# KarelPeeters/kZero

Measured on AMD Instinct MI355X. Metric: self-play NN evals/sec (node), Chess 20x256 ResNet b=256, 1/2/4/8 GPU, higher is better.
Workload: dtype f16; 1 GPU; chess-20x256 attention head, executor batch 256; engines_per_gpu=1, parallelism=dp1 (no collective)

## Files before the change

kzero_amd/csrc/kz_device_weights.hpp:

```cpp
#pragma once

struct DevConv {
    void *w = nullptr;
    float *b = nullptr;
    int cin_p = 0, cout_p = 0, cout = 0, k = 1;
    void *bw = nullptr;
    bool bw2 = false;
    void *bws = nullptr;
    void *sw = nullptr;
};

struct DeviceWeights {
    int device = 0, dtype = 0;
    std::vector<void *> allocs;

    std::vector<DevConv> tower;
    float *post_scale = nullptr, *post_shift = nullptr;

    bool split16 = false;
    float *h32_small = nullptr;
    void *res32_w = nullptr;
    void *res_w_stem = nullptr, *res_w_tower = nullptr;
    float *res_bias = nullptr;
    int32_t *att_idx = nullptr;
// ... 186 lines not shown
                upload_f32(m.att_embedding, &att_embedding))
                return 1;
        } else if (p.tower == Tower::att_valu) {
            std::vector<float> all;
            all.reserve(kz::att_tower_layer_elems(C, m.att_heads, m.att_dk, m.att_dv, m.att_dff) * m.att_layers.size());
            for (auto &l : m.att_layers) {
                all.insert(all.end(), l.qkv.begin(), l.qkv.end());
                all.insert(all.end(), l.out.begin(), l.out.end());
                all.insert(all.end(), l.ff0.begin(), l.ff0.end());
                all.insert(all.end(), l.ff1.begin(), l.ff1.end());
            }
            if (upload_f32(m.att_expand, &att_expand) || upload_f32(m.att_embedding, &att_embedding) || upload_f32(all, &att_layers)) return 1;
        } else if (p.tower == Tower::resident_split16 || p.tower == Tower::resident_f16g) {
            const bool conv_heads = p.heads && m.policy_kind != kz::POLICY_ATTENTION;
            const bool heads = p.heads && !conv_heads;
            const size_t tower_elems = kz::tower_split_weight_elems(C, m.depth, m.c_in, split16);
            std::vector<uint16_t> packed(tower_elems + (heads ? kz::tower_split_heads_weight_elems() : 0) +
                                         (conv_heads ? kz::tower_split_conv_heads_weight_elems(C, split16) : 0));
            const size_t step_elems = (size_t)(split16 ? 2 : 1) * C * 32, stem_elems = kz::tower_split_stem_elems(C, m.c_in, split16),
                         layer_elems = (size_t)9 * (C / 32) * step_elems;
            kz::tower_split_pack_weights(m.tower[0].w.data(), C, m.c_in, hw, true, split16, packed.data());
            for (int l = 0; l < 2 * m.depth; l++)
                kz::tower_split_pack_weights(m.tower[1 + l].w.data(), C, C, hw, false, split16,
                                             packed.data() + stem_elems + layer_elems * l);
            std::vector<float> bias((size_t)(1 + 2 * m.depth + (heads ? 5 : conv_heads ? 1 : 0)) * C);
            for (int l = 0; l < 1 + 2 * m.depth; l++)
                for (int o = 0; o < C; o++) bias[(size_t)l * C + o] = m.tower[l].b[o];
            if (conv_heads) {
                kz::tower_split_pack_conv_heads(m.p_conv0.w.data(), C, split16, packed.data() + tower_elems);
                for (int o = 0; o < C; o++) bias[(size_t)(1 + 2 * m.depth) * C + o] = m.p_conv0.b[o];
                if (!split16) {
                    std::vector<uint16_t> small(kz::tower_split_small_weight16_elems(C));
                    kz::tower_split_pack_small_weights16(m.sh_conv.w.data(), m.sh_conv.cout,
                                                         m.policy_extra_moves ? m.p_extra_conv.w.data() : nullptr,
                                                         m.p_conv1.w.data(), m.policy_conv_channels, C, small.data());
                    if (upload(small.data(), small.size() * 2, (void **)&h32_small)) return 1;
                } else {
                    std::vector<float> small(kz::tower32_small_weight_elems(C));
                    kz::tower32_pack_small_weights(m.sh_conv.w.data(), m.sh_conv.cout,
                                                   m.policy_extra_moves ? m.p_extra_conv.w.data() : nullptr, m.p_conv1.w.data(),
                                                   m.policy_conv_channels, C, small.data());
                    if (upload_f32(small, &h32_small)) return 1;
                }
            }
            if (heads) {
                kz::tower_split_pack_heads(m.p_bulk.w.data(), m.p_bulk.b.data(), m.p_under.w.data(), m.p_under.b.data(),
                                           packed.data() + tower_elems, bias.data() + (size_t)(1 + 2 * m.depth) * C);
                std::vector<int32_t> idx(m.flat_to_att.size());
                for (size_t i = 0; i < idx.size(); i++) idx[i] = (m.flat_to_att[i] / 88) * 96 + m.flat_to_att[i] % 88;
                if (upload(idx.data(), idx.size() * 4, (void **)&att_idx)) return 1;
            }
            if (upload(packed.data(), packed.size() * 2, &res32_w)) return 1;
            if (upload_f32(bias, &res_bias)) return 1;
        } else if (p.tower == Tower::resident_f32) {
            const bool heads32 = kz::tower32_heads_supported((int)m.policy_kind, m.policy_extra_moves,
                                                             m.policy_conv_channels, m.h, m.w, C, m.sh_conv.cout, m.sh_fc0.out);
            const size_t tower_elems = kz::tower32_weight_elems(m.c_in, C, m.depth);
            std::vector<float> packed(tower_elems + (heads32 ? kz::tower32_heads_weight_elems(C) : 0) +
                                      kz::tower32_weight_pad_elems(C), 0.0f);
            const size_t stem_elems = (size_t)9 * ((m.c_in + 15) / 16) * 16 * C, layer_elems = (size_t)9 * C * C;
            kz::tower32_pack_weights(m.tower[0].w.data(), C, m.c_in, true, packed.data());
            for (int l = 0; l < 2 * m.depth; l++)
                kz::tower32_pack_weights(m.tower[1 + l].w.data(), C, C, false, packed.data() + stem_elems + layer_elems * l);
            std::vector<float> bias((size_t)(1 + 2 * m.depth + (heads32 ? 1 : 0)) * C);
            for (int l = 0; l < 1 + 2 * m.depth; l++)
                for (int o = 0; o < C; o++) bias[(size_t)l * C + o] = m.tower[l].b[o];
            if (heads32) {
                kz::tower32_pack_head_weights(m.p_conv0.w.data(), C, packed.data() + tower_elems);
                for (int o = 0; o < C; o++) bias[(size_t)(1 + 2 * m.depth) * C + o] = m.p_conv0.b[o];
                std::vector<float> small(kz::tower32_small_weight_elems(C));
                kz::tower32_pack_small_weights(m.sh_conv.w.data(), m.sh_conv.cout,
                                               m.policy_extra_moves ? m.p_extra_conv.w.data() : nullptr, m.p_conv1.w.data(),
                                               m.policy_conv_channels, C, small.data());
                if (upload_f32(small, &h32_small)) return 1;
            }
            if (upload(packed.data(), packed.size() * 4, &res32_w)) return 1;
            if (upload_f32(bias, &res_bias)) return 1;
        } else if (p.tower == Tower::resident_f16) {
            const int cin_p = round_up(m.c_in, 32);
            const size_t stem_elems = (size_t)9 * 256 * cin_p, layer_elems = (size_t)9 * 256 * 256;
            const size_t head_elems = p.heads ? kz::tower_heads_weight_elems() : 0;
            std::vector<uint16_t> stem(stem_elems), rest(layer_elems * 2 * m.depth + head_elems + kz::tower_weight_pad_elems());
            kz::tower_pack_weights(m.tower[0].w.data(), C, m.c_in, cin_p, stem.data());
            for (int l = 0; l < 2 * m.depth; l++)
                kz::tower_pack_weights(m.tower[1 + l].w.data(), C, C, 256, rest.data() + layer_elems * l);
            std::vector<float> bias((size_t)(1 + 2 * m.depth + (p.heads ? 5 : 0)) * 256);
            for (int l = 0; l < 1 + 2 * m.depth; l++)
                for (int o = 0; o < 256; o++) bias[(size_t)l * 256 + o] = m.tower[l].b[o];
            if (p.heads) {
                kz::tower_pack_heads(m.p_bulk.w.data(), m.p_bulk.b.data(), m.p_under.w.data(), m.p_under.b.data(),
                                     rest.data() + layer_elems * 2 * m.depth, bias.data() + (size_t)(1 + 2 * m.depth) * 256);
                std::vector<int32_t> idx(m.flat_to_att.size());
                for (size_t i = 0; i < idx.size(); i++) idx[i] = (m.flat_to_att[i] / 88) * 96 + m.flat_to_att[i] % 88;
                if (upload(idx.data(), idx.size() * 4, (void **)&att_idx)) return 1;
            }
            if (upload(stem.data(), stem.size() * 2, &res_w_stem)) return 1;
            if (upload(rest.data(), rest.size() * 2, &res_w_tower)) return 1;
            if (upload_f32(bias, &res_bias)) return 1;
        } else {
            tower.resize(m.tower.size());
            const bool on = p.tower == Tower::board_conv_f16, use_board_split = p.tower == Tower::board_conv_split16;
#ifdef KZ_EXPERIMENTS
            conv2 = p.conv2;
            if (conv2) {
                std::vector<int> rowmap;
                std::vector<unsigned short> halo;
                kz::board_conv2_tables(m.h, m.w, rowmap, halo);
                bc_n_halo = (int)halo.size();
                if (upload(rowmap.data(), rowmap.size() * sizeof(int), (void **)&bc_rowmap)) return 1;
                if (upload(halo.data(), halo.size() * sizeof(unsigned short), (void **)&bc_halo)) return 1;
            }
#endif
            for (size_t i = 0; i < m.tower.size(); i++) {
                const bool stem64 = on && i == 0 && !conv2 && m.tower[0].cin <= 64 && m.tower[0].k == 3 &&
                                    kz::board_conv_supported(dtype, m.h, m.w, 64, m.tower[0].cout);
                const bool board = on && kz::board_conv_supported(dtype, m.h, m.w, m.tower[i].cin, m.tower[i].cout);
                if (use_board_split && i == 0 && m.tower[0].cin <= 32 && m.tower[0].k == 3) {
                    stem_split = true;
                    if (upload_board_conv_split(m.tower[0], tower[0], 32)) return 1;
                } else if (use_board_split && i >= 1) {
                    if (upload_board_conv_split(m.tower[i], tower[i])) return 1;
                } else if (stem64) {
                    stem_cin_p = 64;
                    if (upload_board_conv(m.tower[0], tower[0], 64)) return 1;
                } else if (board ? upload_board_conv(m.tower[i], tower[i]) : upload_conv(m.tower[i], tower[i])) {
                    return 1;
                }
            }
        }

        if (upload_f32(m.sh_conv.w, &sh_w0) || upload_f32(m.sh_conv.b, &sh_b0) || upload_f32(m.sh_fc0.w, &sh_w1) ||
            upload_f32(m.sh_fc0.b, &sh_b1) || upload_f32(m.sh_fc1.w, &sh_w2) || upload_f32(m.sh_fc1.b, &sh_b2))
            return 1;
        {
            std::vector<float> wt((size_t)m.sh_fc0.in * m.sh_fc0.out);
            for (int o = 0; o < m.sh_fc0.out; o++)
                for (int i = 0; i < m.sh_fc0.in; i++) wt[(size_t)i * m.sh_fc0.out + o] = m.sh_fc0.w[(size_t)o * m.sh_fc0.in + i];
            if (upload_f32(wt, &sh_w1t)) return 1;
        }

        if (p.tower == Tower::resident_f16 && p.heads) return 0;
        switch (m.policy_kind) {
            case kz::POLICY_ATAXX_CONV:
            case kz::POLICY_CONV:
                if (upload_conv(m.p_conv0, p_conv0)) return 1;
                if (upload_f32(m.p_conv1.w, &p_w1) || upload_f32(m.p_conv1.b, &p_b1)) return 1;
                if (m.policy_extra_moves) {
                    if (upload_f32(m.p_extra_conv.w, &pe_wc) || upload_f32(m.p_extra_conv.b, &pe_bc) ||
                        upload_f32(m.p_extra_fc.w, &pe_wl) || upload_f32(m.p_extra_fc.b, &pe_bl))
                        return 1;
                    if (m.sh_conv.cout == 4 && m.p_extra_conv.cout == 1 && m.p_extra_conv.cin == m.sh_conv.cin) {
                        std::vector<float> w0x(m.sh_conv.w);
                        w0x.insert(w0x.end(), m.p_extra_conv.w.begin(), m.p_extra_conv.w.end());
                        if (upload_f32(w0x, &sh_w0x)) return 1;
                    }
                }
                break;
            case kz::POLICY_ARIMAA: {
                if (upload_conv(m.p_conv0, p_conv0)) return 1;
                if (upload_f32(m.p_conv1.w, &p_w1) || upload_f32(m.p_conv1.b, &p_b1)) return 1;
                if (upload_f32(m.pa_conv.w, &pa_w0) || upload_f32(m.pa_conv.b, &pa_b0) || upload_f32(m.pa_fc0.w, &pa_w1) ||
                    upload_f32(m.pa_fc0.b, &pa_b1) || upload_f32(m.pa_fc1.w, &pa_w2) || upload_f32(m.pa_fc1.b, &pa_b2))
                    return 1;
                std::vector<float> wt((size_t)m.pa_fc0.in * m.pa_fc0.out);
                for (int o = 0; o < m.pa_fc0.out; o++)
                    for (int i = 0; i < m.pa_fc0.in; i++) wt[(size_t)i * m.pa_fc0.out + o] = m.pa_fc0.w[(size_t)o * m.pa_fc0.in + i];
                if (upload_f32(wt, &pa_w1t)) return 1;
                break;
            }
            case kz::POLICY_ATTENTION:
                if (p.att_heads) {
                    const int Q = m.policy_query_channels;
                    std::vector<uint16_t> packed(kz::att_heads_weight_elems(C, Q));
                    std::vector<float> bias((size_t)5 * Q + 16);
                    kz::att_heads_pack(m.p_bulk.w.data(), m.p_bulk.b.data(), m.p_under.w.data(), m.p_under.b.data(), m.sh_conv.w.data(),
                                       m.sh_conv.b.data(), C, Q, m.sh_conv.cout, packed.data(), bias.data());
                    if (upload(packed.data(), packed.size() * 2, &ah_w) || upload_f32(bias, &ah_bias)) return 1;
                } else if (upload_conv(m.p_bulk, p_bulk) || upload_conv(m.p_under, p_under)) {
                    return 1;
                }
                if (upload(m.flat_to_att.data(), m.flat_to_att.size() * 4, (void **)&flat_to_att)) return 1;
                break;
            case kz::POLICY_NONE: break;
            case kz::POLICY_DENSE: {
                int ch = C, ch_p = cp;
                if (m.dense_hidden_channels) {
                    if (upload_conv(m.p_conv0, p_conv0)) return 1;
                    ch = m.dense_hidden_channels;
                    ch_p = p_conv0.cout_p;
                }
                if (m.dense_hidden_size) {
                    if (upload_flat_linear(m.p_fc0, ch, hw, ch_p, p_fc0)) return 1;
                    if (upload_linear(m.p_fc1, p_fc1)) return 1;
                } else {
                    if (upload_flat_linear(m.p_fc1, ch, hw, ch_p, p_fc1)) return 1;
                }
                break;
            }
        }
        return 0;
    }
};

struct WeightsKey {
    const Model *model;
    int device, dtype;
    Tower tower;
    bool heads, att_heads, conv2 = false;
    WeightsKey(const Model *m, int device, int dtype, const PathPlan &p)
        : model(m), device(device), dtype(dtype), tower(p.tower), heads(p.heads && p.tower != Tower::resident_f32), att_heads(p.att_heads) {
#ifdef KZ_EXPERIMENTS
        conv2 = p.conv2;
#endif
    }
    auto fields() const { return std::tie(model, device, dtype, tower, heads, att_heads, conv2); }
    bool operator<(const WeightsKey &o) const { return fields() < o.fields(); }
};
std::mutex g_cache_mutex;
std::map<WeightsKey, std::weak_ptr<DeviceWeights>> g_cache;
```

kzero_amd/csrc/kz_kernels.hpp:

```cpp
#pragma once
#include <vector>
#include <hip/hip_runtime.h>

#include <cstdint>

namespace kz {

inline int round_up(int v, int m) { return (v + m - 1) / m * m; }

struct PackedBoards {
    const uint8_t *bits = nullptr;
    size_t stride = 0;
    const float *scalars = nullptr;
    int n_scalar = 0, n_bool = 0;
    int n_sym = 0;
    const uint8_t *sym = nullptr;
    const int32_t *square_src = nullptr;
};

void launch_encode_packed(int dtype, const PackedBoards &in, int batch, int hw, void *x, int ldx, hipStream_t stream);
void launch_encode_dense(int dtype, const float *nchw, int batch, int c, int hw, void *x, int ldx,
                         hipStream_t stream);

struct ConvArgs {
// ... 210 lines not shown
bool tower32_supported(int dtype, int h, int w, int channels, int depth);
bool tower32_dense3_supported(int policy_kind, int extra_moves, int pc, int h, int w, int channels, int hc, int hs, bool heads);
bool tower32_heads_supported(int policy_kind, int extra_moves, int pc, int h, int w, int channels, int hc, int hs);
bool conv_heads_fit(int nt, int policy_kind, int extra_moves, int pc, int h, int w, int channels, int hc, int hs,
                    size_t scratch_bytes = 0);
constexpr size_t F16_TAIL_SCRATCH_BYTES = 16 * 1024;
size_t tower32_small_weight_elems(int channels);
void tower32_pack_small_weights(const float *sh_w0, int hc, const float *pe_wc , const float *p_w1, int pc,
                                int channels, float *dst);
size_t tower32_heads_weight_elems(int channels);
void tower32_pack_head_weights(const float *oi, int channels, float *dst);
int tower32_boards_per_workgroup(int h, int w, int channels);
size_t tower32_weight_elems(int c_in, int channels, int depth);
size_t tower32_weight_pad_elems(int channels);
void tower32_pack_weights(const float *oihw, int cout, int cin, bool stem, float *dst);
void launch_tower32(const Tower32Args &a, hipStream_t stream);

bool tower_split_supported(int h, int w, int channels, int depth, int c_in, bool split);
int tower_split_boards_per_workgroup(int h, int w, int channels, bool split, int wide_batch = 0);
bool tower_split_wide_supported(int h, int w, int channels, int max_batch);
size_t tower_split_stem_elems(int channels, int c_in, bool split);
size_t tower_split_weight_elems(int channels, int depth, int c_in, bool split);
void tower_split_pack_weights(const float *oihw, int cout, int cin, int hw, bool stem, bool split, uint16_t *dst);
void launch_tower_split(const Tower32Args &a, hipStream_t stream);
bool tower_split_heads_supported(int policy_kind, int query_channels, int policy_len, int h, int w, int channels, int sh_channels,
                                 int sh_size);
size_t tower_split_heads_weight_elems();
void tower_split_pack_heads(const float *w_bulk, const float *b_bulk, const float *w_under, const float *b_under, uint16_t *dst,
                            float *bias5 );
bool tower_split_conv_heads_supported(int policy_kind, int extra_moves, int pc, int h, int w, int channels, int hc, int hs,
                                      bool split, int wide_batch = 0);
size_t tower_split_small_weight16_elems(int channels);
void tower_split_pack_small_weights16(const float *sh_w0, int hc, const float *pe_wc , const float *p_w1, int pc,
                                      int channels, uint16_t *dst);
size_t tower_split_conv_heads_weight_elems(int channels, bool split);
void tower_split_pack_conv_heads(const float *w , int channels, bool split, uint16_t *dst);
void launch_tower_pairs(const Tower32Args &a, bool split, hipStream_t stream);

struct Conv1x1SplitArgs {
    const void *x;
    int ldx;
    const void *weights;
    const float *bias;
    void *y;
    int ldy, M, cin_p, cout_p, relu, group, src_group, src_off;
    bool split;
    const float *pw1 = nullptr, *pb1 = nullptr;
    float *policy = nullptr;
    int policy_len = 0, hw = 0;
};
bool conv1x1_split_supported(int cin_p, int cout_p);
bool conv1x1_policy_epilogue_supported(int cin_p, int cout_p, int cout, int policy_channels);
size_t conv1x1_split_weight_elems(int cin_p, int cout_p, bool split);
void conv1x1_split_pack_weights(const float *w, int cout, int cin, int cout_p, int cin_p, bool split, uint16_t *dst);
void launch_conv1x1_split(const Conv1x1SplitArgs &a, hipStream_t stream);

struct TowerArgs {
    const void *x0;
    int cin_p;
    PackedBoards in;
    const void *w_stem;
    const void *w_tower;
    const float *bias;
    const float *post_scale, *post_shift;
    void *y;
    int batch, h, w, depth;
    int boards_per_wg;
    bool fused_heads;
    const float *sh_w0, *sh_b0, *sh_w1, *sh_b1, *sh_w2, *sh_b2;
    const int32_t *att_idx;
    float *scalars, *policy;
    int *nonfinite_flag;
    int epoch;
    DecodeArgs decode;
    bool prev;
};
bool tower_resident_supported(int dtype, int h, int w, int channels, int depth, int c_in);
bool tower_heads_supported(int policy_kind, int query_channels, int policy_len, int sh_channels, int sh_size);
size_t tower_packed_weight_elems(int cin_p, int depth);
size_t tower_heads_weight_elems();
size_t tower_weight_pad_elems();
void tower_pack_heads(const float *w_bulk, const float *b_bulk, const float *w_under, const float *b_under,
                      uint16_t *dst, float *bias5);
void tower_pack_weights(const float *oihw, int cout, int cin, int cin_p, uint16_t *dst);
void launch_tower_resident(const TowerArgs &a, hipStream_t stream);
size_t tower4_scratch_bytes(int batch);
void launch_tower_resident4(const TowerArgs &a, void *xres, hipStream_t stream);

}
```

kzero_amd/csrc/kz_tower.hip:

```cpp
#include <cstdlib>
#include <type_traits>
#include <vector>

#include "kz_kernels.hpp"
#include "kz_launch.hpp"

namespace kz {

typedef _Float16 h16;
typedef h16 h16x8 __attribute__((ext_vector_type(8)));
typedef h16 h16x4 __attribute__((ext_vector_type(4)));
typedef float f32x4 __attribute__((ext_vector_type(4)));

namespace {

#include "kz_decode_dev.hpp"
#include "kz_encode_dev.hpp"

constexpr int C = 256;
constexpr int RS = C * 2 + 16;
constexpr int URS = 3 * C * 2 + 16;
constexpr int KSTEPS = 72;
constexpr int HEAD_KSTEPS = 5 * 8;
constexpr int POLICY = 1880, LOGIT_LD = 96;
constexpr int TOWER_PF_MAX = 8;

struct TowerDev {
    const h16 *x0;
    const uint4 *w_stem, *w_tower;
    const float *bias, *post_scale, *post_shift;
    h16 *y;
    int cin_p, batch, depth;
    PackedBoards in;
    const float *sh_w0, *sh_b0, *sh_w1, *sh_b1, *sh_w2, *sh_b2;
    const int32_t *att_idx;
    float *scalars, *policy;
    int *nonfinite_flag;
    int epoch;
    DecodeDev dec;
};

template <int NB>
struct Layout {
    static constexpr int M = NB * 64;
    static constexpr int MT = M / 16;
    static constexpr bool LINE_TILES = NB == 2;
    static constexpr int BPAD = LINE_TILES ? 128 : 0;
    static constexpr int BOARD = 64 * RS + BPAD;
    static constexpr int TS = LINE_TILES ? 8 * RS : 16 * RS;
    static constexpr int IMG = NB * BOARD;
    static constexpr int X_OFF = 0;
    static constexpr int Y_OFF = IMG;
    static constexpr int Z_OFF = 2 * IMG;
    static_assert(Z_OFF % 256 == 0, "zero rows keep the slot pattern of the image rows");
    static constexpr int S_OFF = Z_OFF + 16 * RS;
    static constexpr int TOWER_BYTES = S_OFF + M * 64;
    static constexpr int U_OFF = Z_OFF;
    static constexpr int ACT_OFF = U_OFF + 16 * URS;
    static constexpr int HID_OFF = ACT_OFF + NB * 256 * 4;
    static constexpr int HEADS_BYTES = HID_OFF + NB * 32 * 4;
    static constexpr int LOG_OFF = Y_OFF;
    static constexpr int BYTES = TOWER_BYTES > HEADS_BYTES ? TOWER_BYTES : HEADS_BYTES;
    static_assert(NB * 64 * LOGIT_LD * 4 <= IMG, "logits fit the Y region");
    static constexpr int row_off(int b, int p) { return b * BOARD + p * RS; }
    static_assert(BYTES <= 160 * 1024, "LDS budget");
};

constexpr int SG_VALU = 0x2, SG_SALU = 0x4, SG_MFMA = 0x8, SG_VMEM_READ = 0x20, SG_DS_READ = 0x100;

template <int NB, bool HEADS, int PF, bool WIDE = false, bool PREV = false>
__global__ __launch_bounds__(256, 1) void kz_tower_resident(TowerDev a) {
    using L = Layout<NB>;
    constexpr int M = L::M, MT = L::MT;
    static_assert(PF <= TOWER_PF_MAX, "the refills past the end of the stream must land in its padding");
    extern __shared__ __attribute__((aligned(16))) unsigned char lds[];

    const int tid = threadIdx.x;
    const int wave = __builtin_amdgcn_readfirstlane(tid >> 6);
    const int lane = tid & 63;
    const int fr = lane & 15, kq = lane >> 4;
    const int board0 = blockIdx.x * NB;
    const int layers = 2 * a.depth;
    const int total_ksteps = layers * KSTEPS + (HEADS ? HEAD_KSTEPS : 0);
    const int bias_rows = layers + (HEADS ? 5 : 0);

    const uint4 *wp = a.w_tower + wave * 256 + lane;
    auto wload_prev = [&](int gk, int nt) __attribute__((always_inline)) { return wp[(size_t)gk * 1024 + nt * 64]; };
    typedef const __attribute__((address_space(1))) unsigned char *gptr;
    gptr wk = (gptr)a.w_tower + wave * 4096;
    const unsigned wlane = lane * 16;
    auto wload = [&](gptr k, int nt) __attribute__((always_inline)) {
        typedef unsigned u32x4 __attribute__((ext_vector_type(4)));
        return __builtin_bit_cast(uint4, *reinterpret_cast<const __attribute__((address_space(1))) u32x4 *>(k + wlane + nt * 1024));
    };
    uint4 wreg[PF][4];
#pragma unroll
    for (int s = 0; s < PF; s++) {
        const int g = s < total_ksteps ? s : total_ksteps - 1;
#pragma unroll
        for (int nt = 0; nt < 4; nt++) wreg[s][nt] = PREV ? wload_prev(g, nt) : wload(wk + s * 16384, nt);
    }
    wk += PF * 16384;
    int g = 0;
    auto ring_take = [&](int stage, h16x8 (&af)[4]) __attribute__((always_inline)) {
#pragma unroll
        for (int nt = 0; nt < 4; nt++) af[nt] = *reinterpret_cast<const h16x8 *>(&wreg[stage][nt]);
#ifndef KZ_TW_NO_WLOAD
        if constexpr (PREV) {
            const int gn = g + PF < total_ksteps ? g + PF : total_ksteps - 1;
#pragma unroll
            for (int nt = 0; nt < 4; nt++) wreg[stage][nt] = wload_prev(gn, nt);
        } else {
#pragma unroll
            for (int nt = 0; nt < 4; nt++) wreg[stage][nt] = wload(wk, nt);
        }
#endif
        wk += 16384;
        if constexpr (!PREV) asm("" : "+s"(wk));
    };

    const int sc = WIDE ? a.cin_p >> 5 : 1;
    const int stem_off = WIDE ? L::Y_OFF : L::S_OFF, srow = 64 * sc, spieces = 4 * sc;
    for (int id = tid; id < 16 * RS / 16; id += 256)
// ... 29 lines not shown
        for (int nt = 0; nt < 4; nt++)
#pragma unroll
            for (int mt = 0; mt < MT; mt++) acc[nt][mt] = bias_next[nt];
    };
    f32x4 post_s[4], post_t[4];
#pragma unroll
    for (int nt = 0; nt < 4; nt++) {
        post_s[nt] = f32x4{1.f, 1.f, 1.f, 1.f};
        post_t[nt] = f32x4{0.f, 0.f, 0.f, 0.f};
    }

    auto relu4 = [](f32x4 v) {
        typedef int i32x4 __attribute__((ext_vector_type(4)));
        i32x4 b = __builtin_bit_cast(i32x4, v);
#pragma unroll
        for (int j = 0; j < 4; j++) b[j] = b[j] > 0 ? b[j] : 0;
        return __builtin_bit_cast(f32x4, b);
    };
    auto to_h4 = [](f32x4 v) { return h16x4{(h16)v[0], (h16)v[1], (h16)v[2], (h16)v[3]}; };

    const int lane_row = L::LINE_TILES ? (fr >> 3) * L::BOARD + (fr & 7) * RS : fr * RS;
    const int epi_base = lane_row + (wave * 64 + kq * 4) * 2;
    auto epilogue = [&](int dst_off, auto relu, auto residual, auto post) __attribute__((always_inline)) {
#pragma unroll
        for (int nt = 0; nt < 4; nt++) {
            h16x4 rx[MT];
            if constexpr (decltype(residual)::value) {
#pragma unroll
                for (int mt = 0; mt < MT; mt++)
                    rx[mt] = *reinterpret_cast<const h16x4 *>(lds + L::X_OFF + epi_base + mt * L::TS + nt * 32);
            }
#pragma unroll
            for (int mt = 0; mt < MT; mt++) {
                const int off = epi_base + mt * L::TS + nt * 32;
                f32x4 v = acc[nt][mt];
                if constexpr (decltype(relu)::value) v = relu4(v);
                if constexpr (decltype(residual)::value) {
#pragma unroll
                    for (int j = 0; j < 4; j++) v[j] += (float)rx[mt][j];
                }
                if constexpr (decltype(post)::value) v = v * post_s[nt] + post_t[nt];
                *reinterpret_cast<h16x4 *>(lds + dst_off + off) = to_h4(v);
            }
        }
    };
    constexpr std::true_type YES{};
    constexpr std::false_type NO{};

    const bool x_is0 = (lane & 7) == 0, x_is7 = (lane & 7) == 7, yo_is0 = (lane & 8) == 0, yo_is1 = !yo_is0;
    auto tap_ok = [&](int mt, int dy, int dx) __attribute__((always_inline)) {
        const bool kill_x = (dx < 0 && x_is0) || (dx > 0 && x_is7);
        if constexpr (L::LINE_TILES) return !(kill_x || (dy < 0 && mt == 0) || (dy > 0 && mt == MT - 1));
        else return !(kill_x || ((mt & 3) == 0 && dy < 0 && yo_is0) || ((mt & 3) == 3 && dy > 0 && yo_is1));
    };

    fetch_bias(0);
    init_acc();
    fetch_bias(1);
    for (int ks = 0; ks < 9 * sc; ks++) {
        const int tap = WIDE ? ks / sc : ks, chunk = ks - tap * sc;
        const int dy = tap / 3 - 1, dx = tap % 3 - 1;
        h16x8 af[4];
#pragma unroll
        for (int nt = 0; nt < 4; nt++) {
            const uint4 t = a.w_stem[((ks * 4 + wave) * 4 + nt) * 64 + lane];
            af[nt] = *reinterpret_cast<const h16x8 *>(&t);
        }
#pragma unroll
        for (int mt = 0; mt < MT; mt++) {
            const bool ok = tap_ok(mt, dy, dx);
            const int p = L::LINE_TILES ? (fr >> 3) * 64 + mt * 8 + (fr & 7) : mt * 16 + fr;
            const int off = ok ? stem_off + (p + dy * 8 + dx) * srow + chunk * 64 + kq * 16 : L::Z_OFF + kq * 16;
            const h16x8 bf = *reinterpret_cast<const h16x8 *>(lds + off);
#pragma unroll
            for (int nt = 0; nt < 4; nt++)
                acc[nt][mt] = __builtin_amdgcn_mfma_f32_16x16x32_f16(af[nt], bf, acc[nt][mt], 0, 0, 0);
        }
    }
    epilogue(L::X_OFF, NO, NO, NO);
    __syncthreads();

    const int kq_off = 256 * (kq & 1) + 128 * (kq >> 1);
    const int frag_base = lane_row + kq_off;
    auto tap_rows = [&](int tap, int src_off, int (&T)[MT]) __attribute__((always_inline)) {
        const int dy = tap / 3 - 1, dx = tap % 3 - 1;
        const int shifted = frag_base + src_off + (dy * 8 + dx) * RS;
        const int zrow = L::Z_OFF + ((fr + dy * 8 + dx) & 15) * RS + kq_off;
        const int zrow_odd = L::LINE_TILES ? L::Z_OFF + ((fr + dy * 8 + dx + 8) & 15) * RS + kq_off : zrow;
        if constexpr (PREV) {
#pragma unroll
            for (int mt = 0; mt < MT; mt++) T[mt] = tap_ok(mt, dy, dx) ? shifted + mt * L::TS : ((mt & 1) ? zrow_odd : zrow);
        } else {
            int z0 = zrow, z1 = zrow_odd;
            asm("" : "+v"(z0), "+v"(z1));
            const bool kill_x = ((dx < 0) & x_is0) | ((dx > 0) & x_is7);
#pragma unroll
            for (int mt = 0; mt < MT; mt++) {
                bool kill;
                if constexpr (L::LINE_TILES) kill = kill_x | ((dy < 0) & (mt == 0)) | ((dy > 0) & (mt == MT - 1));
                else kill = kill_x | (((mt & 3) == 0) & (dy < 0) & yo_is0) | (((mt & 3) == 3) & (dy > 0) & yo_is1);
                T[mt] = kill ? ((mt & 1) ? z1 : z0) : shifted + mt * L::TS;
            }
        }
    };

    h16x8 bf[2][MT];
    auto conv_line = [&](auto dy_tag, int src_off, int dx_lo, int dx_hi, int tap_after) __attribute__((always_inline)) {
        constexpr int DY = decltype(dy_tag)::value;
        constexpr int LO = L::LINE_TILES && DY < 0 ? 1 : 0, HI = L::LINE_TILES && DY > 0 ? MT - 1 : MT, NT_ = HI - LO;
        int T[MT], Tn[MT];
        tap_rows((DY + 1) * 3 + dx_lo + 1, src_off, T);
#pragma nounroll
        for (int dx = dx_lo; dx < dx_hi; dx++) {
            tap_rows(dx + 1 < dx_hi ? (DY + 1) * 3 + dx + 2 : tap_after, src_off, Tn);
#pragma unroll
            for (int ch = 0; ch < 8; ch++) {
                const int stage = ch & (PF - 1), cur = ch & 1, nxt = cur ^ 1;
#ifndef KZ_TW_NO_DSREAD
#pragma unroll
                for (int mt = 0; mt < MT; mt++) {
                    if (ch < 7) {
                        if (mt >= LO && mt < HI) bf[nxt][mt] = *reinterpret_cast<const h16x8 *>(lds + T[mt] + (ch + 1) * 16);
                    } else {
                        bf[nxt][mt] = *reinterpret_cast<const h16x8 *>(lds + Tn[mt]);
                    }
                }
#endif
                h16x8 af[4];
                ring_take(stage, af);
#pragma unroll
                for (int nt = 0; nt < 4; nt++)
#pragma unroll
                    for (int mt = LO; mt < HI; mt++)
                        acc[nt][mt] = __builtin_amdgcn_mfma_f32_16x16x32_f16(af[nt], bf[cur][mt], acc[nt][mt], 0, 0, 0);
                constexpr int NR_LAST = MT;
                const int nr = ch < 7 ? NT_ : NR_LAST;
#pragma unroll
                for (int i = 0; i < 4; i++) {
                    __builtin_amdgcn_sched_group_barrier(SG_MFMA, 1, 0);
                    __builtin_amdgcn_sched_group_barrier(SG_VMEM_READ, 1, 0);
                }
#pragma unroll
                for (int i = 0; i < MT; i++) {
                    if (i < nr) {
                        __builtin_amdgcn_sched_group_barrier(SG_MFMA, 1, 0);
                        __builtin_amdgcn_sched_group_barrier(SG_DS_READ, 1, 0);
                    }
                }
                constexpr int N_FREE = 4 * NT_ - (NT_ + 4), N_ALU = PREV ? 0 : N_FREE < 20 ? N_FREE : 20;
                if (ch == 0) {
#pragma unroll
                    for (int i = 0; i < N_ALU; i++) {
                        __builtin_amdgcn_sched_group_barrier(SG_MFMA, 1, 0);
                        __builtin_amdgcn_sched_group_barrier(SG_VALU | SG_SALU, 2, 0);
                    }
                    __builtin_amdgcn_sched_group_barrier(SG_MFMA, 4 * NT_ - (NT_ + 4) - N_ALU, 0);
                } else if (ch < 7) {
                    __builtin_amdgcn_sched_group_barrier(SG_MFMA, 4 * NT_ - (NT_ + 4), 0);
                } else {
                    __builtin_amdgcn_sched_group_barrier(SG_MFMA, 4 * NT_ - (NR_LAST + 4), 0);
                }
                __builtin_amdgcn_sched_barrier(0);
                g++;
            }
#pragma unroll
            for (int mt = 0; mt < MT; mt++) T[mt] = Tn[mt];
        }
    };
    constexpr std::integral_constant<int, -1> DY_UP{};
    constexpr std::integral_constant<int, 0> DY_MID{};
    constexpr std::integral_constant<int, 1> DY_DOWN{};
    auto conv_prime = [&](int src_off, int tap) __attribute__((always_inline)) {
        int T[MT];
        tap_rows(tap, src_off, T);
#pragma unroll
        for (int mt = 0; mt < MT; mt++) bf[0][mt] = *reinterpret_cast<const h16x8 *>(lds + T[mt]);
    };
    auto conv_3x3 = [&](int src_off) __attribute__((always_inline)) {
        conv_prime(src_off, 0);
        conv_line(DY_UP, src_off, -1, 2, 3);
        conv_line(DY_MID, src_off, -1, 2, 6);
        conv_line(DY_DOWN, src_off, -1, 2, 8);
    };
    auto conv_1x1 = [&](int src_off) __attribute__((always_inline)) {
        conv_prime(src_off, 4);
        conv_line(DY_MID, src_off, 0, 1, 4);
    };

    for (int layer = 1; layer <= layers; layer++) {
        const bool is_b = (layer & 1) == 0;
        init_acc();
        fetch_bias(layer + 1);
        if (layer == layers) {
#pragma unroll
            for (int nt = 0; nt < 4; nt++) {
                const int oc = wave * 64 + nt * 16 + kq * 4;
                post_s[nt] = *reinterpret_cast<const f32x4 *>(a.post_scale + oc);
                post_t[nt] = *reinterpret_cast<const f32x4 *>(a.post_shift + oc);
            }
        }
        conv_3x3(is_b ? L::Y_OFF : L::X_OFF);
        if (!is_b) epilogue(L::Y_OFF, YES, NO, NO);
        else if (layer != layers) epilogue(L::X_OFF, YES, YES, NO);
        else epilogue(L::X_OFF, YES, YES, YES);
        __syncthreads();
    }

    if constexpr (!HEADS) {
        for (int id = tid; id < M * 32; id += 256) {
            const int p = id >> 5, c16 = id & 31;
            const int board = board0 + (p >> 6);
            if (board < a.batch) {
                const uint4 v = *reinterpret_cast<const uint4 *>(lds + L::X_OFF + L::row_off(p >> 6, p & 63) + c16 * 16);
                *reinterpret_cast<uint4 *>(a.y + ((size_t)board0 * 64 + p) * C + c16 * 8) = v;
            }
        }
    } else {
        {
            float *act = reinterpret_cast<float *>(lds + L::ACT_OFF);
            for (int o = tid; o < NB * 256; o += 256) {
                const int b = o >> 8, c4 = (o >> 6) & 3, p = o & 63;
                const unsigned char *row = lds + L::X_OFF + L::row_off(b, p);
                const float *w = a.sh_w0 + c4 * C;
                float s = a.sh_b0[c4];
#pragma unroll 4
                for (int i = 0; i < C; i += 8) {
                    const h16x8 xv = *reinterpret_cast<const h16x8 *>(row + i * 2);
                    const f32x4 w0 = *reinterpret_cast<const f32x4 *>(w + i), w1 = *reinterpret_cast<const f32x4 *>(w + i + 4);
#pragma unroll
                    for (int j = 0; j < 4; j++) s += (float)xv[j] * w0[j] + (float)xv[4 + j] * w1[j];
                }
                if (!(fabsf(s) <= 3.0e38f) && a.nonfinite_flag && board0 + b < a.batch)
                    *reinterpret_cast<volatile int *>(a.nonfinite_flag) = a.epoch;
                act[o] = fmaxf(s, 0.0f);
            }
        }

        {
            const int tb = L::X_OFF + L::row_off(NB == 2 ? fr >> 3 : 0, 56 + (fr & 7)) + kq_off;
            for (int s = 0; s < 3; s++) {
                f32x4 ua[4];
#pragma unroll
                for (int nt = 0; nt < 4; nt++) ua[nt] = bias_next[nt];
                fetch_bias(layers + 2 + s);
#pragma unroll
                for (int ch = 0; ch < 8; ch++) {
                    const h16x8 bf = *reinterpret_cast<const h16x8 *>(lds + tb + ch * 16);
                    h16x8 af[4];
                    ring_take(ch & (PF - 1), af);
#pragma unroll
                    for (int nt = 0; nt < 4; nt++)
                        ua[nt] = __builtin_amdgcn_mfma_f32_16x16x32_f16(af[nt], bf, ua[nt], 0, 0, 0);
                    g++;
                }
                if (NB == 2 || fr < 8) {
#pragma unroll
                    for (int nt = 0; nt < 4; nt++)
                        *reinterpret_cast<h16x4 *>(lds + L::U_OFF + fr * URS + (256 * s + wave * 64 + nt * 16 + kq * 4) * 2) =
                            to_h4(ua[nt]);
                }
            }
        }

        init_acc();
        fetch_bias(layers + 5);
        conv_1x1(L::X_OFF);
        epilogue(L::Y_OFF, NO, NO, NO);

        init_acc();
        conv_1x1(L::X_OFF);
// ... 52 lines not shown
        }
        __syncthreads();
        {
            const float inv = 1.0f / sqrtf((float)C);
#pragma unroll
            for (int ii = 0; ii < IT; ii++)
#pragma unroll
                for (int jt = 0; jt < 6; jt++) {
                    const int i = (it0 + ii) * 16 + fr, j = jt * 16 + kq * 4;
                    *reinterpret_cast<f32x4 *>(lds + L::LOG_OFF + ((hb * 64 + i) * LOGIT_LD + j) * 4) = la[ii][jt] * inv;
                }
        }
        const bool decode = a.dec.move_offsets != nullptr;
        float *raw = reinterpret_cast<float *>(lds + L::ACT_OFF);
        if (tid < NB * 5) {
            const int b = tid / 5, k = tid % 5;
            const float *hid = reinterpret_cast<const float *>(lds + L::HID_OFF) + b * 32;
            float s = a.sh_b2[k];
            for (int i = 0; i < 32; i++) s += a.sh_w2[k * 32 + i] * hid[i];
            if (decode) raw[b * 8 + k] = s;
            else if (board0 + b < a.batch) a.scalars[(size_t)(board0 + b) * 5 + k] = s;
        }
        __syncthreads();
        if (decode) {
            if (wave < NB && board0 + wave < a.batch) {
                const float *lg = reinterpret_cast<const float *>(lds + L::LOG_OFF) + wave * 64 * LOGIT_LD;
                float *stage = reinterpret_cast<float *>(lds + L::X_OFF + L::row_off(wave, 0));
                decode_board_wave(a.dec, board0 + wave, lane, raw + wave * 8, stage, 64 * RS / 4,
                                  [&](int idx) { return lg[a.att_idx[idx]]; });
            }
        } else {
            for (int b = 0; b < NB; b++) {
                if (board0 + b >= a.batch) break;
                const float *lg = reinterpret_cast<const float *>(lds + L::LOG_OFF) + b * 64 * LOGIT_LD;
                float *pol = a.policy + (size_t)(board0 + b) * POLICY;
                for (int k = tid; k < POLICY; k += 256) pol[k] = lg[a.att_idx[k]];
            }
        }
    }
}

#ifndef KZ_PF_NB1
#define KZ_PF_NB1 4
#endif
#ifndef KZ_PF_NB2
#define KZ_PF_NB2 4
#endif
constexpr int PF_NB1 = KZ_PF_NB1, PF_NB2 = KZ_PF_NB2;

void pack_1x1(const float *w, uint16_t *dst) {
    static const int kq_base[4] = {0, 128, 64, 192};
    for (int chunk = 0; chunk < 8; chunk++)
        for (int wave = 0; wave < 4; wave++)
            for (int nt = 0; nt < 4; nt++)
                for (int lane = 0; lane < 64; lane++)
                    for (int j = 0; j < 8; j++) {
                        const int oc = 64 * wave + 16 * nt + (lane & 15);
                        const int ch = 8 * chunk + kq_base[lane >> 4] + j;
                        const _Float16 hv = (_Float16)w[(size_t)oc * 256 + ch];
                        uint16_t bits;
                        __builtin_memcpy(&bits, &hv, 2);
                        dst[((((size_t)chunk * 4 + wave) * 4 + nt) * 64 + lane) * 8 + j] = bits;
                    }
}

}

bool tower_resident_supported(int dtype, int h, int w, int channels, int depth, int c_in) {
    return dtype == 1 && h == 8 && w == 8 && channels == C && depth >= 1 && c_in >= 1 && c_in <= 224;
}

bool tower_heads_supported(int policy_kind, int query_channels, int policy_len, int sh_channels, int sh_size) {
    return policy_kind == 2 && query_channels == C && policy_len == POLICY && sh_channels == 4 && sh_size == 32;
}

size_t tower_packed_weight_elems(int cin_p, int depth) {
    return (size_t)9 * C * cin_p + (size_t)2 * depth * 9 * C * C;
}

size_t tower_heads_weight_elems() { return (size_t)HEAD_KSTEPS * 16 * 1024 / 2; }

size_t tower_weight_pad_elems() { return (size_t)TOWER_PF_MAX * 16 * 1024 / 2; }

void tower_pack_weights(const float *oihw, int cout, int cin, int cin_p, uint16_t *dst) {
    const int nchunk = cin_p / 32;
    static const int kq_base[4] = {0, 128, 64, 192};
    for (int tap = 0; tap < 9; tap++)
        for (int chunk = 0; chunk < nchunk; chunk++)
            for (int wave = 0; wave < 4; wave++)
                for (int nt = 0; nt < 4; nt++)
                    for (int lane = 0; lane < 64; lane++)
                        for (int j = 0; j < 8; j++) {
                            const int oc = 64 * wave + 16 * nt + (lane & 15);
                            const int kq = lane >> 4;
                            const int ch = cin_p == 256 ? 8 * chunk + kq_base[kq] + j : 32 * chunk + 8 * kq + j;
                            float v = 0.0f;
                            if (oc < cout && ch < cin) v = oihw[((size_t)oc * cin + ch) * 9 + tap];
                            const _Float16 hv = (_Float16)v;
                            uint16_t bits;
                            __builtin_memcpy(&bits, &hv, 2);
                            dst[(((((size_t)tap * nchunk + chunk) * 4 + wave) * 4 + nt) * 64 + lane) * 8 + j] = bits;
                        }
}

void tower_pack_heads(const float *w_bulk , const float *b_bulk, const float *w_under ,
                      const float *b_under, uint16_t *dst, float *bias5) {
    const size_t pass = (size_t)8 * 16 * 1024 / 2;
    std::vector<float> tmp((size_t)256 * 256);
    for (int s = 0; s < 3; s++) {
        for (int q = 0; q < 256; q++) {
            for (int c = 0; c < 256; c++) tmp[(size_t)q * 256 + c] = w_under[(size_t)(3 * q + s) * 256 + c];
            bias5[s * 256 + q] = b_under[3 * q + s];
        }
        pack_1x1(tmp.data(), dst + pass * s);
    }
    pack_1x1(w_bulk, dst + pass * 3);
    pack_1x1(w_bulk + (size_t)256 * 256, dst + pass * 4);
    for (int q = 0; q < 256; q++) {
        bias5[3 * 256 + q] = b_bulk[q];
        bias5[4 * 256 + q] = b_bulk[256 + q];
    }
}

namespace {
template <auto Kernel>
void launch_instance(const TowerDev &d, int grid, int bytes, hipStream_t stream) {
    allow_dynamic_lds<Kernel>(bytes);
    Kernel<<<grid, 256, bytes, stream>>>(d);
}
}

void launch_tower_resident(const TowerArgs &t, hipStream_t stream) {
    TowerDev d{};
    d.x0 = static_cast<const h16 *>(t.x0);
    d.w_stem = static_cast<const uint4 *>(t.w_stem);
    d.w_tower = static_cast<const uint4 *>(t.w_tower);
    d.bias = t.bias;
    d.post_scale = t.post_scale;
    d.post_shift = t.post_shift;
    d.y = static_cast<h16 *>(t.y);
    d.cin_p = t.cin_p;
    d.batch = t.batch;
    d.depth = t.depth;
    d.in = t.in;
    d.sh_w0 = t.sh_w0; d.sh_b0 = t.sh_b0; d.sh_w1 = t.sh_w1; d.sh_b1 = t.sh_b1; d.sh_w2 = t.sh_w2; d.sh_b2 = t.sh_b2;
    d.att_idx = t.att_idx;
    d.scalars = t.scalars;
    d.policy = t.policy;
    d.nonfinite_flag = t.nonfinite_flag;
    d.epoch = t.epoch;
    d.dec = decode_dev(t.decode, t.fused_heads, POLICY);
    const bool heads = t.fused_heads;
#ifdef KZ_EXPERIMENTS
    if (t.prev) {
        const int grid = (t.batch + 1) / 2;
        if (t.cin_p > 32) {
            if (heads) launch_instance<kz_tower_resident<2, true, PF_NB2, true, true>>(d, grid, Layout<2>::BYTES, stream);
            else launch_instance<kz_tower_resident<2, false, PF_NB2, true, true>>(d, grid, Layout<2>::BYTES, stream);
        } else if (t.boards_per_wg == 1) {
            if (heads) launch_instance<kz_tower_resident<1, true, PF_NB1, false, true>>(d, t.batch, Layout<1>::BYTES, stream);
            else launch_instance<kz_tower_resident<1, false, PF_NB1, false, true>>(d, t.batch, Layout<1>::BYTES, stream);
        } else {
            if (heads) launch_instance<kz_tower_resident<2, true, PF_NB2, false, true>>(d, grid, Layout<2>::BYTES, stream);
            else launch_instance<kz_tower_resident<2, false, PF_NB2, false, true>>(d, grid, Layout<2>::BYTES, stream);
        }
        return;
    }
#endif
    if (t.cin_p > 32) {
        const int grid = (t.batch + 1) / 2;
        if (heads) launch_instance<kz_tower_resident<2, true, PF_NB2, true>>(d, grid, Layout<2>::BYTES, stream);
        else launch_instance<kz_tower_resident<2, false, PF_NB2, true>>(d, grid, Layout<2>::BYTES, stream);
    } else if (t.boards_per_wg == 1) {
        if (heads) launch_instance<kz_tower_resident<1, true, PF_NB1>>(d, t.batch, Layout<1>::BYTES, stream);
        else launch_instance<kz_tower_resident<1, false, PF_NB1>>(d, t.batch, Layout<1>::BYTES, stream);
    } else {
        const int grid = (t.batch + 1) / 2;
        if (heads) launch_instance<kz_tower_resident<2, true, PF_NB2>>(d, grid, Layout<2>::BYTES, stream);
        else launch_instance<kz_tower_resident<2, false, PF_NB2>>(d, grid, Layout<2>::BYTES, stream);
    }
}

}
```

Baseline: 520,500 evals/s.

## Reuse each LDS activation fragment across three vertical taps in line-tile 3x3 conv

Result: faster. 548,500 evals/s, median of 6 (+5.4%).

```diff
diff --git a/kzero_amd/csrc/kz_device_weights.hpp b/kzero_amd/csrc/kz_device_weights.hpp
--- a/kzero_amd/csrc/kz_device_weights.hpp
+++ b/kzero_amd/csrc/kz_device_weights.hpp
@@ -292,8 +292,12 @@
             const size_t head_elems = p.heads ? kz::tower_heads_weight_elems() : 0;
             std::vector<uint16_t> stem(stem_elems), rest(layer_elems * 2 * m.depth + head_elems + kz::tower_weight_pad_elems());
             kz::tower_pack_weights(m.tower[0].w.data(), C, m.c_in, cin_p, stem.data());
+            bool tap_major = false;
+#ifdef KZ_EXPERIMENTS
+            tap_major = p.nb4;
+#endif
             for (int l = 0; l < 2 * m.depth; l++)
-                kz::tower_pack_weights(m.tower[1 + l].w.data(), C, C, 256, rest.data() + layer_elems * l);
+                kz::tower_pack_weights(m.tower[1 + l].w.data(), C, C, 256, rest.data() + layer_elems * l, tap_major);
             std::vector<float> bias((size_t)(1 + 2 * m.depth + (p.heads ? 5 : 0)) * 256);
             for (int l = 0; l < 1 + 2 * m.depth; l++)
                 for (int o = 0; o < 256; o++) bias[(size_t)l * 256 + o] = m.tower[l].b[o];
@@ -416,14 +420,15 @@
     const Model *model;
     int device, dtype;
     Tower tower;
-    bool heads, att_heads, conv2 = false;
+    bool heads, att_heads, conv2 = false, nb4 = false;
     WeightsKey(const Model *m, int device, int dtype, const PathPlan &p)
         : model(m), device(device), dtype(dtype), tower(p.tower), heads(p.heads && p.tower != Tower::resident_f32), att_heads(p.att_heads) {
 #ifdef KZ_EXPERIMENTS
         conv2 = p.conv2;
+        nb4 = p.nb4;
 #endif
     }
-    auto fields() const { return std::tie(model, device, dtype, tower, heads, att_heads, conv2); }
+    auto fields() const { return std::tie(model, device, dtype, tower, heads, att_heads, conv2, nb4); }
     bool operator<(const WeightsKey &o) const { return fields() < o.fields(); }
 };
 std::mutex g_cache_mutex;
diff --git a/kzero_amd/csrc/kz_kernels.hpp b/kzero_amd/csrc/kz_kernels.hpp
--- a/kzero_amd/csrc/kz_kernels.hpp
+++ b/kzero_amd/csrc/kz_kernels.hpp
@@ -316,7 +316,7 @@
 size_t tower_weight_pad_elems();
 void tower_pack_heads(const float *w_bulk, const float *b_bulk, const float *w_under, const float *b_under,
                       uint16_t *dst, float *bias5);
-void tower_pack_weights(const float *oihw, int cout, int cin, int cin_p, uint16_t *dst);
+void tower_pack_weights(const float *oihw, int cout, int cin, int cin_p, uint16_t *dst, bool tap_major = false);
 void launch_tower_resident(const TowerArgs &a, hipStream_t stream);
 size_t tower4_scratch_bytes(int batch);
 void launch_tower_resident4(const TowerArgs &a, void *xres, hipStream_t stream);
diff --git a/kzero_amd/csrc/kz_tower.hip b/kzero_amd/csrc/kz_tower.hip
--- a/kzero_amd/csrc/kz_tower.hip
+++ b/kzero_amd/csrc/kz_tower.hip
@@ -39,6 +39,14 @@
     int epoch;
     DecodeDev dec;
 };
+
+template <int I, int N, class F>
+__device__ __forceinline__ void static_for(F &&f) {
+    if constexpr (I < N) {
+        f(std::integral_constant<int, I>{});
+        static_for<I + 1, N>(f);
+    }
+}
 
 template <int NB>
 struct Layout {
@@ -234,8 +242,7 @@
 
     const int kq_off = 256 * (kq & 1) + 128 * (kq >> 1);
     const int frag_base = lane_row + kq_off;
-    auto tap_rows = [&](int tap, int src_off, int (&T)[MT]) __attribute__((always_inline)) {
-        const int dy = tap / 3 - 1, dx = tap % 3 - 1;
+    auto tap_rows = [&](int dy, int dx, int src_off, int (&T)[MT]) __attribute__((always_inline)) {
         const int shifted = frag_base + src_off + (dy * 8 + dx) * RS;
         const int zrow = L::Z_OFF + ((fr + dy * 8 + dx) & 15) * RS + kq_off;
         const int zrow_odd = L::LINE_TILES ? L::Z_OFF + ((fr + dy * 8 + dx + 8) & 15) * RS + kq_off : zrow;
@@ -248,34 +255,39 @@
             const bool kill_x = ((dx < 0) & x_is0) | ((dx > 0) & x_is7);
 #pragma unroll
             for (int mt = 0; mt < MT; mt++) {
-                bool kill;
-                if constexpr (L::LINE_TILES) kill = kill_x | ((dy < 0) & (mt == 0)) | ((dy > 0) & (mt == MT - 1));
-                else kill = kill_x | (((mt & 3) == 0) & (dy < 0) & yo_is0) | (((mt & 3) == 3) & (dy > 0) & yo_is1);
+                bool kill = kill_x;
+                if constexpr (!L::LINE_TILES) kill = kill_x | (((mt & 3) == 0) & (dy < 0) & yo_is0) | (((mt & 3) == 3) & (dy > 0) & yo_is1);
                 T[mt] = kill ? ((mt & 1) ? z1 : z0) : shifted + mt * L::TS;
             }
         }
     };
 
     h16x8 bf[2][MT];
-    auto conv_line = [&](auto dy_tag, int src_off, int dx_lo, int dx_hi, int tap_after) __attribute__((always_inline)) {
-        constexpr int DY = decltype(dy_tag)::value;
-        constexpr int LO = L::LINE_TILES && DY < 0 ? 1 : 0, HI = L::LINE_TILES && DY > 0 ? MT - 1 : MT, NT_ = HI - LO;
-        int T[MT], Tn[MT];
-        tap_rows((DY + 1) * 3 + dx_lo + 1, src_off, T);
+    constexpr auto tile_lo = [](int dy) { return L::LINE_TILES && dy < 0 ? 1 : 0; };
+    constexpr auto tile_hi = [](int dy) { return L::LINE_TILES && dy > 0 ? MT - 1 : MT; };
+
+    auto conv_plain = [&](auto ndy_tag, int src_off, int dx_lo, int dx_hi) __attribute__((always_inline)) {
+        constexpr int NDY = decltype(ndy_tag)::value, DY0 = NDY == 3 ? -1 : 0;
+        int T[NDY][MT], Tn[NDY][MT];
+#pragma unroll
+        for (int i = 0; i < NDY; i++) tap_rows(DY0 + i, dx_lo, src_off, T[i]);
+#pragma unroll
+        for (int mt = tile_lo(DY0); mt < tile_hi(DY0); mt++) bf[0][mt] = *reinterpret_cast<const h16x8 *>(lds + T[0][mt]);
 #pragma nounroll
         for (int dx = dx_lo; dx < dx_hi; dx++) {
-            tap_rows(dx + 1 < dx_hi ? (DY + 1) * 3 + dx + 2 : tap_after, src_off, Tn);
-#pragma unroll
-            for (int ch = 0; ch < 8; ch++) {
-                const int stage = ch & (PF - 1), cur = ch & 1, nxt = cur ^ 1;
+#pragma unroll
+            for (int i = 0; i < NDY; i++) tap_rows(DY0 + i, dx + 1 < dx_hi ? dx + 1 : dx, src_off, Tn[i]);
+            static_for<0, 8 * NDY>([&](auto s_tag) __attribute__((always_inline)) {
+                constexpr int s = decltype(s_tag)::value, ch = s / NDY, i = s % NDY, dy = DY0 + i;
+                constexpr int stage = s & (PF - 1), cur = s & 1, nxt = cur ^ 1;
+                constexpr int lo = tile_lo(dy), hi = tile_hi(dy), nt_ = hi - lo;
+                constexpr int in_ = (i + 1) % NDY, chn = i + 1 < NDY ? ch : ch + 1;
+                constexpr int lon = tile_lo(DY0 + in_), hin = tile_hi(DY0 + in_), nr = hin - lon;
 #ifndef KZ_TW_NO_DSREAD
 #pragma unroll
                 for (int mt = 0; mt < MT; mt++) {
-                    if (ch < 7) {
-                        if (mt >= LO && mt < HI) bf[nxt][mt] = *reinterpret_cast<const h16x8 *>(lds + T[mt] + (ch + 1) * 16);
-                    } else {
-                        bf[nxt][mt] = *reinterpret_cast<const h16x8 *>(lds + Tn[mt]);
-                    }
+                    if (mt >= lon && mt < hin)
+                        bf[nxt][mt] = *reinterpret_cast<const h16x8 *>(lds + (chn < 8 ? T[in_][mt] + chn * 16 : Tn[in_][mt]));
                 }
 #endif
                 h16x8 af[4];
@@ -283,61 +295,104 @@
 #pragma unroll
                 for (int nt = 0; nt < 4; nt++)
 #pragma unroll
-                    for (int mt = LO; mt < HI; mt++)
-                        acc[nt][mt] = __builtin_amdgcn_mfma_f32_16x16x32_f16(af[nt], bf[cur][mt], acc[nt][mt], 0, 0, 0);
-                constexpr int NR_LAST = MT;
-                const int nr = ch < 7 ? NT_ : NR_LAST;
-#pragma unroll
-                for (int i = 0; i < 4; i++) {
+                    for (int mt = 0; mt < MT; mt++)
+                        if (mt >= lo && mt < hi)
+                            acc[nt][mt] = __builtin_amdgcn_mfma_f32_16x16x32_f16(af[nt], bf[cur][mt], acc[nt][mt], 0, 0, 0);
+#pragma unroll
+                for (int j = 0; j < 4; j++) {
                     __builtin_amdgcn_sched_group_barrier(SG_MFMA, 1, 0);
                     __builtin_amdgcn_sched_group_barrier(SG_VMEM_READ, 1, 0);
                 }
 #pragma unroll
-                for (int i = 0; i < MT; i++) {
-                    if (i < nr) {
+                for (int j = 0; j < MT; j++) {
+                    if (j < nr) {
                         __builtin_amdgcn_sched_group_barrier(SG_MFMA, 1, 0);
                         __builtin_amdgcn_sched_group_barrier(SG_DS_READ, 1, 0);
                     }
                 }
-                constexpr int N_FREE = 4 * NT_ - (NT_ + 4), N_ALU = PREV ? 0 : N_FREE < 20 ? N_FREE : 20;
-                if (ch == 0) {
-#pragma unroll
-                    for (int i = 0; i < N_ALU; i++) {
+                constexpr int n_free = 4 * nt_ - (nr + 4), n_alu = PREV || s != 0 ? 0 : n_free < 20 ? n_free : 20;
+#pragma unroll
+                for (int j = 0; j < 20; j++) {
+                    if (j < n_alu) {
                         __builtin_amdgcn_sched_group_barrier(SG_MFMA, 1, 0);
                         __builtin_amdgcn_sched_group_barrier(SG_VALU | SG_SALU, 2, 0);
                     }
-                    __builtin_amdgcn_sched_group_barrier(SG_MFMA, 4 * NT_ - (NT_ + 4) - N_ALU, 0);
-                } else if (ch < 7) {
-                    __builtin_amdgcn_sched_group_barrier(SG_MFMA, 4 * NT_ - (NT_ + 4), 0);
-                } else {
-                    __builtin_amdgcn_sched_group_barrier(SG_MFMA, 4 * NT_ - (NR_LAST + 4), 0);
-                }
+                }
+                __builtin_amdgcn_sched_group_barrier(SG_MFMA, n_free - n_alu, 0);
                 __builtin_amdgcn_sched_barrier(0);
                 g++;
-            }
+            });
+#pragma unroll
+            for (int i = 0; i < NDY; i++)
+#pragma unroll
+                for (int mt = 0; mt < MT; mt++) T[i][mt] = Tn[i][mt];
+        }
+    };
+
+    auto conv_3x3_lines = [&](int src_off) __attribute__((always_inline)) {
+        static_assert(!L::LINE_TILES || MT == 8, "one tile per board line");
+        int T[MT], Tn[MT];
+        tap_rows(0, -1, src_off, T);
+#pragma unroll
+        for (int mt = 0; mt < MT; mt++) bf[0][mt] = *reinterpret_cast<const h16x8 *>(lds + T[mt]);
+#pragma nounroll
+        for (int dx = -1; dx < 2; dx++) {
+            tap_rows(0, dx < 1 ? dx + 1 : dx, src_off, Tn);
+            static_for<0, 8>([&](auto ch_tag) __attribute__((always_inline)) {
+                constexpr int ch = decltype(ch_tag)::value, cur = ch & 1, nxt = cur ^ 1;
+#ifndef KZ_TW_NO_DSREAD
+#pragma unroll
+                for (int mt = 0; mt < MT; mt++)
+                    bf[nxt][mt] = *reinterpret_cast<const h16x8 *>(lds + (ch < 7 ? T[mt] + (ch + 1) * 16 : Tn[mt]));
+#endif
+                static_for<0, 3>([&](auto i_tag) __attribute__((always_inline)) {
+                    constexpr int i = decltype(i_tag)::value, dy = i - 1, stage = (ch * 3 + i) & (PF - 1);
+                    constexpr int lo = tile_lo(dy), hi = tile_hi(dy), nt_ = hi - lo;
+                    h16x8 af[4];
+                    ring_take(stage, af);
+#pragma unroll
+                    for (int nt = 0; nt < 4; nt++)
+#pragma unroll
+                        for (int mt = 0; mt < MT; mt++)
+                            if (mt >= lo && mt < hi)
+                                acc[nt][mt] = __builtin_amdgcn_mfma_f32_16x16x32_f16(af[nt], bf[cur][mt + dy], acc[nt][mt], 0, 0, 0);
+#pragma unroll
+                    for (int j = 0; j < 4; j++) {
+                        __builtin_amdgcn_sched_group_barrier(SG_MFMA, 1, 0);
+                        __builtin_amdgcn_sched_group_barrier(SG_VMEM_READ, 1, 0);
+                    }
+                    constexpr int nr = i == 0 ? MT : 0;
+#pragma unroll
+                    for (int j = 0; j < MT; j++) {
+                        if (j < nr) {
+                            __builtin_amdgcn_sched_group_barrier(SG_MFMA, 1, 0);
+                            __builtin_amdgcn_sched_group_barrier(SG_DS_READ, 1, 0);
+                        }
+                    }
+                    constexpr int n_free = 4 * nt_ - (nr + 4), n_alu = ch == 0 && i == 0 ? n_free : 0;
+#pragma unroll
+                    for (int j = 0; j < 4 * MT; j++) {
+                        if (j < n_alu) {
+                            __builtin_amdgcn_sched_group_barrier(SG_MFMA, 1, 0);
+                            __builtin_amdgcn_sched_group_barrier(SG_VALU | SG_SALU, 2, 0);
+                        }
+                    }
+                    __builtin_amdgcn_sched_group_barrier(SG_MFMA, n_free - n_alu, 0);
+                    __builtin_amdgcn_sched_barrier(0);
+                    g++;
+                });
+            });
 #pragma unroll
             for (int mt = 0; mt < MT; mt++) T[mt] = Tn[mt];
         }
     };
-    constexpr std::integral_constant<int, -1> DY_UP{};
-    constexpr std::integral_constant<int, 0> DY_MID{};
-    constexpr std::integral_constant<int, 1> DY_DOWN{};
-    auto conv_prime = [&](int src_off, int tap) __attribute__((always_inline)) {
-        int T[MT];
-        tap_rows(tap, src_off, T);
-#pragma unroll
-        for (int mt = 0; mt < MT; mt++) bf[0][mt] = *reinterpret_cast<const h16x8 *>(lds + T[mt]);
-    };
+    constexpr std::integral_constant<int, 3> THREE_ROWS{};
+    constexpr std::integral_constant<int, 1> ONE_ROW{};
     auto conv_3x3 = [&](int src_off) __attribute__((always_inline)) {
-        conv_prime(src_off, 0);
-        conv_line(DY_UP, src_off, -1, 2, 3);
-        conv_line(DY_MID, src_off, -1, 2, 6);
-        conv_line(DY_DOWN, src_off, -1, 2, 8);
-    };
-    auto conv_1x1 = [&](int src_off) __attribute__((always_inline)) {
-        conv_prime(src_off, 4);
-        conv_line(DY_MID, src_off, 0, 1, 4);
-    };
+        if constexpr (L::LINE_TILES && !PREV) conv_3x3_lines(src_off);
+        else conv_plain(THREE_ROWS, src_off, -1, 2);
+    };
+    auto conv_1x1 = [&](int src_off) __attribute__((always_inline)) { conv_plain(ONE_ROW, src_off, 0, 1); };
 
     for (int layer = 1; layer <= layers; layer++) {
         const bool is_b = (layer & 1) == 0;
@@ -556,11 +611,13 @@
 
 size_t tower_weight_pad_elems() { return (size_t)TOWER_PF_MAX * 16 * 1024 / 2; }
 
-void tower_pack_weights(const float *oihw, int cout, int cin, int cin_p, uint16_t *dst) {
+void tower_pack_weights(const float *oihw, int cout, int cin, int cin_p, uint16_t *dst, bool tap_major) {
     const int nchunk = cin_p / 32;
+    const bool rows_inner = cin_p == 256 && !tap_major;
     static const int kq_base[4] = {0, 128, 64, 192};
     for (int tap = 0; tap < 9; tap++)
-        for (int chunk = 0; chunk < nchunk; chunk++)
+        for (int chunk = 0; chunk < nchunk; chunk++) {
+            const size_t kstep = rows_inner ? ((size_t)(tap % 3) * 8 + chunk) * 3 + tap / 3 : (size_t)tap * nchunk + chunk;
             for (int wave = 0; wave < 4; wave++)
                 for (int nt = 0; nt < 4; nt++)
                     for (int lane = 0; lane < 64; lane++)
@@ -573,8 +630,9 @@
                             const _Float16 hv = (_Float16)v;
                             uint16_t bits;
                             __builtin_memcpy(&bits, &hv, 2);
-                            dst[(((((size_t)tap * nchunk + chunk) * 4 + wave) * 4 + nt) * 64 + lane) * 8 + j] = bits;
+                            dst[(((kstep * 4 + wave) * 4 + nt) * 64 + lane) * 8 + j] = bits;
                         }
+        }
 }
 
 void tower_pack_heads(const float *w_bulk , const float *b_bulk, const float *w_under ,
```
